# ardaduz/deep-video-mvs

Hardware: AMD Instinct MI355X
Metric: depth frames/sec/GPU @ 320x256x64 planes (fusionnet); rel-L1 vs ref (higher is better)
Workload: dtype f32

## Files before the change

### deep-video-mvs_amd/csrc/direct_conv.hip

```cpp
#include <stdlib.h>

#include "dvmvs_device.h"

namespace dvmvs {

typedef float float4v __attribute__((ext_vector_type(4)));

struct DirectConvArgs {
  const float* x;
  const float* packed;
  const float* bias;
  float* dst;
  float* dst_nhwc;
  long long x_batch_stride, dst_batch_stride;
  int B, C_in, C_out, H, W, OH, OW;
  int act;
  int n_groups;
  int packed_groups;
  int n_chunks;
  int tiles_x;
  int vec4;
};

#ifdef DVMVS_SWEEP_TRACE
// ... 313 lines not shown
#pragma clang fp contract(off)
  if (act == 1) return fmaxf(v, 0.0f);
  if (act == 2 || act == 3) {
    const float s = 1.0f / (1.0f + expf(-v));
    return act == 2 ? s : 1.0f / (p0 * s + p1);
  }
  return v;
}

template <int PX>
__global__ __launch_bounds__(256) void conv_head_kernel(const float* __restrict__ x, const float* __restrict__ w, const float* __restrict__ bias,
                                                        float* __restrict__ dst, long long x_batch_stride, long long dst_batch_stride, int C, int H,
                                                        int W, int act, float p0, float p1) {
  constexpr int SL = 256 / PX;
  __shared__ float s_part[SL][PX];
  const int px = threadIdx.x % PX, slice = threadIdx.x / PX;
  const int HW = H * W;
  const int p = blockIdx.x * PX + px, b = blockIdx.y;
  const int y = p / W, xx = p - y * W;
  const int per = (C + SL - 1) / SL;
  const int c_lo = slice * per, c_hi = min(C, c_lo + per);
  float sum = 0.0f;
  if (p < HW) {
    int off[9];
    bool in[9];
#pragma unroll
    for (int t = 0; t < 9; ++t) {
      const int yy = y + t / 3 - 1, xs = xx + t % 3 - 1;
      in[t] = yy >= 0 && yy < H && xs >= 0 && xs < W;
      off[t] = in[t] ? yy * W + xs : 0;
    }
    const float* xb = x + static_cast<size_t>(b) * x_batch_stride;
#pragma unroll 2
    for (int c = c_lo; c < c_hi; ++c) {
      const float* plane = xb + static_cast<size_t>(c) * HW;
      float v[9];
#pragma unroll
      for (int t = 0; t < 9; ++t) v[t] = in[t] ? plane[off[t]] : 0.0f;
#pragma unroll
      for (int t = 0; t < 9; ++t) sum = fmaf(v[t], w[c * 9 + t], sum);
    }
  }
  s_part[slice][px] = sum;
  __syncthreads();
  if (slice == 0 && p < HW) {
    float total = s_part[0][px];
#pragma unroll
    for (int s = 1; s < SL; ++s) total += s_part[s][px];
    if (bias) total += bias[0];
    dst[static_cast<size_t>(b) * dst_batch_stride + p] = head_activation(total, act, p0, p1);
  }
}

struct DirectConvShape {
  int MW, MT, NT, PW, KS;
};
constexpr DirectConvShape kDcShapes[4] = {{16, 5, 2, 4, 2}, {8, 5, 2, 1, 8}, {16, 5, 1, 1, 8}, {8, 5, 1, 1, 8}};
constexpr int kDcCUs = 256;

inline int direct_conv_choose(int B, int C_in, int C_out, int H, int W, int K, int S) {
  if (B <= 0 || C_in <= 0 || C_out <= 0 || C_out % 16 != 0 || (K != 3 && K != 5) || (S != 1 && S != 2) || H <= 0 || W <= 0) return 0;
  if (S == 2 && (H % 2 != 0 || W % 2 != 0)) return 0;
  const int OH = H / S, OW = W / S;
#if defined(DVMVS_SWEEP_TUNING)
  const char* f = getenv("DVMVS_DC_SHAPE");
  const int forced = f ? atoi(f) : 0;
#else
  const int forced = 0;
#endif
  int best = 0;
  double best_fill = 0.0;
  for (int id = 1; id <= 4; ++id) {
    const DirectConvShape& s = kDcShapes[id - 1];
    const int tile_h = s.PW * (16 / s.MW), tile_w = s.MW * s.MT;
    if (OW % tile_w != 0 || C_out % (16 * s.NT) != 0) continue;
    if (forced == id) return id;
    if (forced) continue;
    const long long groups = static_cast<long long>(OW / tile_w) * ((OH + tile_h - 1) / tile_h) * (C_out / (16 * s.NT)) * B;
    const double fill = static_cast<double>(groups) / static_cast<double>(kDcCUs * ((groups + kDcCUs - 1) / kDcCUs));
    if (fill > best_fill + 1e-9) {
      best_fill = fill;
      best = id;
    }
  }
  return best;
}

template <class Cfg>
int launch_direct_conv(DirectConvArgs a, hipStream_t stream) {
  static bool configured[64] = {};
  constexpr size_t lds = sizeof(float) * Cfg::LDS_FLOATS;
  if (lds > 64 * 1024) {
    int device = 0;
    DVMVS_RETURN_IF_HIP(hipGetDevice(&device));
    const bool tracked = device >= 0 && device < 64;
    if (!tracked || !configured[device]) {
      DVMVS_RETURN_IF_HIP(hipFuncSetAttribute(reinterpret_cast<const void*>(direct_conv_kernel<Cfg>), hipFuncAttributeMaxDynamicSharedMemorySize,
                                              static_cast<int>(lds)));
      if (tracked) configured[device] = true;
    }
  }
  a.n_chunks = (a.n_groups + Cfg::KS * Cfg::G - 1) / (Cfg::KS * Cfg::G);
  a.tiles_x = a.OW / Cfg::TILE_W;
  const int tiles_y = (a.OH + Cfg::TILE_H - 1) / Cfg::TILE_H;
  const dim3 grid(a.tiles_x * tiles_y, a.C_out / (16 * Cfg::NTILE), a.B), block(Cfg::NT);
  hipLaunchKernelGGL((direct_conv_kernel<Cfg>), grid, block, lds, stream, a);
// ... 22 lines not shown

extern "C" size_t dvmvs_direct_conv_packed_bytes(int C_out, int C_in, int kernel_size, int n_tile) {
  if (C_out <= 0 || C_in <= 0 || (n_tile != 1 && n_tile != 2) || C_out % (16 * n_tile) != 0 || (kernel_size != 3 && kernel_size != 5)) return 0;
  const size_t Q = (n_tile * kernel_size + 3) / 4;
  return sizeof(float) * (C_out / (16 * n_tile)) * dvmvs::dc_packed_groups(C_in) * kernel_size * Q * 256;
}

extern "C" int dvmvs_direct_conv_pack(const float* weight, float* packed, int C_out, int C_in, int kernel_size, int n_tile, dvmvs_stream_t stream) {
  if (!weight || !packed) return DVMVS_EINVAL;
  const size_t bytes = dvmvs_direct_conv_packed_bytes(C_out, C_in, kernel_size, n_tile);
  if (bytes == 0) return DVMVS_EUNSUPPORTED;
  const long long total = static_cast<long long>(bytes / sizeof(float));
  hipLaunchKernelGGL(dvmvs::direct_conv_pack_kernel, dim3(static_cast<unsigned int>((total + 255) / 256)), dim3(256), 0, static_cast<hipStream_t>(stream),
                     weight, packed, C_out, C_in, kernel_size, n_tile, dvmvs::dc_packed_groups(C_in), total);
  return dvmvs::launch_status();
}

extern "C" int dvmvs_direct_conv_fwd(const float* x, long long x_batch_stride, const float* packed, int n_tile, const float* bias, float* dst,
                                     long long dst_batch_stride, int B, int C_in, int H, int W, int C_out, int kernel_size, int stride, int activation,
                                     dvmvs_stream_t stream) {
  return dvmvs_direct_conv_dual_fwd(x, x_batch_stride, packed, n_tile, bias, dst, dst_batch_stride, nullptr, B, C_in, H, W, C_out, kernel_size, stride, activation,
                                    stream);
}

extern "C" int dvmvs_direct_conv_dual_fwd(const float* x, long long x_batch_stride, const float* packed, int n_tile, const float* bias, float* dst,
                                          long long dst_batch_stride, float* dst_nhwc, int B, int C_in, int H, int W, int C_out, int kernel_size, int stride,
                                          int activation, dvmvs_stream_t stream) {
  using namespace dvmvs;
  if (!x || !packed || !dst || B <= 0) return DVMVS_EINVAL;
  if (activation != 0 && activation != 1) return DVMVS_EUNSUPPORTED;
  const int id = direct_conv_choose(B, C_in, C_out, H, W, kernel_size, stride);
  if (id == 0) return DVMVS_EUNSUPPORTED;
  if (kDcShapes[id - 1].NT != n_tile) return DVMVS_EINVAL;
  DirectConvArgs a;
  a.x = x; a.packed = packed; a.bias = bias; a.dst = dst; a.dst_nhwc = dst_nhwc;
  a.B = B; a.C_in = C_in; a.C_out = C_out; a.H = H; a.W = W; a.OH = H / stride; a.OW = W / stride;
  a.x_batch_stride = x_batch_stride ? x_batch_stride : static_cast<long long>(C_in) * H * W;
  a.dst_batch_stride = dst_batch_stride ? dst_batch_stride : static_cast<long long>(C_out) * a.OH * a.OW;
  if (a.x_batch_stride < static_cast<long long>(C_in) * H * W || a.dst_batch_stride < static_cast<long long>(C_out) * a.OH * a.OW) return DVMVS_EINVAL;
  if (W % 4 != 0 || a.x_batch_stride % 4 != 0 || (reinterpret_cast<uintptr_t>(x) & 15) != 0) return DVMVS_EUNSUPPORTED;
  if (static_cast<long long>(C_in + 64) * H * W * 4 >= (1LL << 31)) return DVMVS_EUNSUPPORTED;
  a.act = activation;
  a.n_groups = (C_in + 3) / 4;
  a.packed_groups = dc_packed_groups(C_in);
  a.vec4 = (a.OW % 4 == 0 && (a.OH * a.OW) % 4 == 0 && a.dst_batch_stride % 4 == 0 && (reinterpret_cast<uintptr_t>(dst) & 15) == 0) ? 1 : 0;
  a.n_chunks = 0; a.tiles_x = 0;
  hipStream_t s = static_cast<hipStream_t>(stream);
  if (kernel_size == 3) return stride == 1 ? launch_direct_conv_shape<3, 1>(id, a, s) : launch_direct_conv_shape<3, 2>(id, a, s);
  return stride == 1 ? launch_direct_conv_shape<5, 1>(id, a, s) : launch_direct_conv_shape<5, 2>(id, a, s);
}

extern "C" int dvmvs_conv_head_fwd(const float* x, long long x_batch_stride, const float* weight, const float* bias, float* dst,
                                   long long dst_batch_stride, int B, int C_in, int H, int W, int activation, float p0, float p1, dvmvs_stream_t stream) {
  using namespace dvmvs;
  if (!x || !weight || !dst || B <= 0 || C_in <= 0 || H <= 0 || W <= 0) return DVMVS_EINVAL;
  if (activation < 0 || activation > 3) return DVMVS_EINVAL;
  const long long HW = static_cast<long long>(H) * W;
  if (x_batch_stride == 0) x_batch_stride = HW * C_in;
  if (dst_batch_stride == 0) dst_batch_stride = HW;
  hipStream_t s = static_cast<hipStream_t>(stream);
  if (HW >= 16384) {
    hipLaunchKernelGGL((conv_head_kernel<64>), dim3(static_cast<unsigned int>((HW + 63) / 64), B), dim3(256), 0, s, x, weight, bias, dst, x_batch_stride,
                       dst_batch_stride, C_in, H, W, activation, p0, p1);
  } else {
    hipLaunchKernelGGL((conv_head_kernel<16>), dim3(static_cast<unsigned int>((HW + 15) / 16), B), dim3(256), 0, s, x, weight, bias, dst, x_batch_stride,
                       dst_batch_stride, C_in, H, W, activation, p0, p1);
  }
  return launch_status();
}

#ifdef DVMVS_SWEEP_TRACE
extern "C" int dvmvs_debug_direct_conv_trace(unsigned long long* host, int waves) {
  if (waves > dvmvs::kDcTraceWaves) waves = dvmvs::kDcTraceWaves;
  return static_cast<int>(hipMemcpyFromSymbol(host, HIP_SYMBOL(dvmvs::g_dc_trace), sizeof(unsigned long long) * dvmvs::kDcTraceWords * waves));
}
#endif
```

### deep-video-mvs_amd/dvmvs/hip/_capi.py

```python
import ctypes
import os
import threading

import torch

_HERE = os.path.dirname(os.path.abspath(__file__))
LIB_PATH = os.environ.get("DVMVS_HIP_LIB", os.path.normpath(os.path.join(_HERE, "..", "..", "lib", "libdvmvs_hip.so")))

ABI_VERSION = 11
MAX_MEASUREMENTS = 8
MAX_DEPTH_LEVELS = 256
LAYOUT_NCHW, LAYOUT_NHWC = 0, 1

_c_fp = ctypes.c_void_p
_c_fpp = ctypes.POINTER(ctypes.c_void_p)
_c_int = ctypes.c_int
_c_dbl = ctypes.c_double
_c_stream = ctypes.c_void_p
_c_f3 = ctypes.POINTER(ctypes.c_float)

SIGNATURES = {
    "dvmvs_abi_version": (_c_int, []),
    "dvmvs_build_arch": (ctypes.c_char_p, []),
    "dvmvs_error_string": (ctypes.c_char_p, [_c_int]),
    "dvmvs_trace_marker": (_c_int, [_c_stream]),
    "dvmvs_host_pointer_device_visible": (_c_int, [ctypes.c_void_p]),
    "dvmvs_cost_volume_workspace_bytes": (ctypes.c_size_t, [_c_int, _c_int, _c_int, _c_int, _c_int]),
    "dvmvs_sweep_matrices": (_c_int, [_c_fp, _c_fpp, _c_fp, _c_fp, _c_fp, _c_int, _c_int, _c_stream]),
    "dvmvs_cost_volume_fwd": (_c_int, [_c_fp, _c_fpp, _c_fp, _c_fp, _c_fp,
                                       _c_int, _c_int, _c_int, _c_int, _c_int, _c_int,
                                       _c_dbl, _c_dbl, _c_int, _c_int, _c_int, _c_fp, ctypes.c_size_t, _c_stream]),
    "dvmvs_sweep_plan_stats": (_c_int, [_c_fp, _c_fp, _c_int, _c_int, _c_int, _c_int, _c_int, _c_dbl, _c_dbl, _c_int,
                                        ctypes.POINTER(ctypes.c_longlong)]),
    "dvmvs_sweep_select_variant": (_c_int, [_c_fp, _c_fp, _c_int, _c_int, _c_int, _c_int, _c_int, _c_dbl, _c_dbl]),
    "dvmvs_sweep_work_list_bytes": (ctypes.c_size_t, [_c_int, _c_int, _c_int, _c_int]),
    "dvmvs_sweep_work_list": (_c_int, [_c_fp, _c_fp, _c_int, _c_int, _c_int, _c_int, _c_int, _c_dbl, _c_dbl, _c_int, _c_fp, ctypes.c_size_t]),
    "dvmvs_sweep_plan": (_c_int, [_c_fp, _c_fp, _c_int, _c_int, _c_int, _c_int, _c_int, _c_dbl, _c_dbl, _c_int, _c_fp, ctypes.c_size_t]),
    "dvmvs_sweep_plan6": (_c_int, [_c_fp, _c_fp, _c_int, _c_int, _c_int, _c_int, _c_int, _c_dbl, _c_dbl, _c_fp, ctypes.c_size_t]),
    "dvmvs_nchw_to_nhwc": (_c_int, [_c_fp, _c_fp, _c_int, _c_int, _c_int, _c_int, _c_stream]),
    "dvmvs_copy_batch": (_c_int, [_c_fpp, _c_fpp, ctypes.POINTER(ctypes.c_longlong), _c_int, _c_stream]),
    "dvmvs_sweep_mfma_estimate": (_c_int, [_c_fp, _c_fp, _c_int, _c_int, _c_int, _c_int, _c_int, _c_dbl, _c_dbl, ctypes.POINTER(ctypes.c_double)]),
    "dvmvs_cost_volume_planned_fwd": (_c_int, [_c_fp, _c_fpp, _c_fp, _c_fp, _c_fp,
                                               _c_int, _c_int, _c_int, _c_int, _c_int, _c_int,
                                               _c_dbl, _c_dbl, _c_int, _c_int, _c_int, _c_fp, ctypes.c_size_t, _c_fp, _c_stream]),
    "dvmvs_cost_volume_bwd": (_c_int, [_c_fp, _c_fp, _c_fpp, _c_fp, _c_fp, _c_fp, _c_fpp,
                                       _c_int, _c_int, _c_int, _c_int, _c_int, _c_int,
                                       _c_dbl, _c_dbl, _c_stream]),
    "dvmvs_hidden_warp_fwd": (_c_int, [_c_fp, _c_fp, _c_fp, _c_fp, _c_fp, _c_int, _c_int, _c_int, _c_int, _c_int, _c_stream]),
    "dvmvs_hidden_warp_bwd": (_c_int, [_c_fp, _c_fp, _c_fp, _c_fp, _c_fp, _c_int, _c_int, _c_int, _c_int, _c_stream]),
    "dvmvs_relative_pose": (_c_int, [_c_fp, _c_fp, _c_fp, _c_int, _c_stream]),
    "dvmvs_lstm_gates_fwd": (_c_int, [_c_fp, _c_fp, _c_fp, _c_fp, _c_int, _c_int, _c_int, _c_int, _c_stream]),
    "dvmvs_lstm_gates_bwd": (_c_int, [_c_fp, _c_fp, _c_fp, _c_fp, _c_fp, _c_fp, _c_int, _c_int, _c_int, _c_int, _c_stream]),
    "dvmvs_lstm_gates_partials_fwd": (_c_int, [_c_fp, _c_int, _c_fp, _c_fp, _c_fp, _c_int, _c_int, _c_int, _c_int, _c_stream]),
    "dvmvs_bottleneck_conv_packed_bytes": (ctypes.c_size_t, [_c_int, _c_int]),
    "dvmvs_bottleneck_conv_pack": (_c_int, [_c_fp, _c_fp, _c_int, _c_int, _c_stream]),
    "dvmvs_bottleneck_conv_splits": (_c_int, [_c_int] * 6),
    "dvmvs_bottleneck_conv_fwd": (_c_int, [_c_fp, _c_fp, _c_fp] + [_c_int] * 6 + [_c_stream]),
    "dvmvs_bottleneck_conv_up2x_fwd": (_c_int, [_c_fp, _c_fp, _c_fp] + [_c_int] * 5 + [_c_stream]),
    "dvmvs_direct_conv_tile": (_c_int, [_c_int] * 7),
    "dvmvs_direct_conv_packed_bytes": (ctypes.c_size_t, [_c_int] * 4),
    "dvmvs_direct_conv_pack": (_c_int, [_c_fp, _c_fp, _c_int, _c_int, _c_int, _c_int, _c_stream]),
    "dvmvs_direct_conv_fwd": (_c_int, [_c_fp, ctypes.c_longlong, _c_fp, _c_int, _c_fp, _c_fp, ctypes.c_longlong] + [_c_int] * 8 + [_c_stream]),
    "dvmvs_direct_conv_dual_fwd": (_c_int, [_c_fp, ctypes.c_longlong, _c_fp, _c_int, _c_fp, _c_fp, ctypes.c_longlong, _c_fp] + [_c_int] * 8 + [_c_stream]),
    "dvmvs_pointwise_conv_supported": (_c_int, [_c_int] * 7),
    "dvmvs_pointwise_conv_packed_bytes": (ctypes.c_size_t, [_c_int] * 2),
    "dvmvs_pointwise_conv_pack": (_c_int, [_c_fp, _c_fp, _c_int, _c_int, _c_stream]),
    "dvmvs_pointwise_conv_fwd": (_c_int, [_c_fp, ctypes.c_longlong, _c_fp, _c_fp, _c_fp, ctypes.c_longlong, _c_int, _c_fp, ctypes.c_longlong] + [_c_int] * 7 + [_c_stream]),
    "dvmvs_conv_head_fwd": (_c_int, [_c_fp, ctypes.c_longlong, _c_fp, _c_fp, _c_fp, ctypes.c_longlong] + [_c_int] * 5 + [ctypes.c_float, ctypes.c_float, _c_stream]),
    "dvmvs_partial_sums_bias_act_fwd": (_c_int, [_c_fp, _c_int, _c_fp, ctypes.c_longlong, _c_fp, _c_int, _c_int, _c_int, _c_int, _c_stream]),
    "dvmvs_depth_reproject_fwd": (_c_int, [_c_fp, _c_fp, _c_fp, _c_fp, _c_fp, _c_fp, _c_int,
                                           _c_int, _c_int, _c_int, _c_stream]),
    "dvmvs_bias_act_fwd": (_c_int, [_c_fp, _c_fp, ctypes.c_longlong, _c_fp, _c_fp, _c_int, _c_int, _c_int, _c_int, _c_int, _c_int,
                                    ctypes.c_float, ctypes.c_float, _c_stream]),
    "dvmvs_bias_act_inplace": (_c_int, [_c_fp, _c_fp, _c_fp, _c_int, _c_int, _c_int, _c_int, _c_int, _c_int, _c_stream]),
    "dvmvs_conv_bias_act_fwd": (_c_int, [_c_fp, _c_fp, _c_fp, _c_fp, ctypes.c_longlong] + [_c_int] * 9 + [_c_stream]),
    "dvmvs_upsample2x_fwd": (_c_int, [_c_fp, _c_fp, ctypes.c_longlong, _c_fp, _c_int, _c_int, _c_int, _c_int, _c_int, _c_stream]),
    "dvmvs_upsample2x_pair_fwd": (_c_int, [_c_fp, _c_fp, ctypes.c_longlong, _c_int, _c_fp, _c_fp, ctypes.c_longlong, _c_fp, _c_int, _c_int, _c_int, _c_int, _c_int, _c_stream]),
    "dvmvs_upsample2x_bwd": (_c_int, [_c_fp, _c_fp, _c_int, _c_int, _c_int, _c_int, _c_stream]),
    "dvmvs_depthwise_conv_bwd_workspace_bytes": (ctypes.c_size_t, [_c_int] * 6),
    "dvmvs_depthwise_conv_bwd": (_c_int, [_c_fp, _c_fp, _c_fp, _c_fp, _c_fp, _c_fp, _c_int, _c_int, _c_int, _c_int, _c_int, _c_int, _c_stream]),
    "dvmvs_depth_reproject_lowres_fwd": (_c_int, [_c_fp, _c_fp, _c_fp, _c_fp, _c_fp, _c_fp, _c_int, _c_int, _c_int, _c_int, _c_stream]),
    "dvmvs_depth_reproject_estimate_fwd": (_c_int, [_c_fp, _c_fp, _c_fp, _c_fp, _c_fp, _c_fp, _c_int, _c_int, _c_int, _c_int, _c_stream]),
    "dvmvs_tsdf_integrate": (_c_int, [_c_fp, _c_fp, _c_fp, _c_int, _c_int, _c_int, ctypes.c_float, ctypes.c_float, ctypes.c_float,
                                      ctypes.c_float, _c_fp, _c_fp, _c_fp, _c_fp, _c_int, _c_int, ctypes.c_float, ctypes.c_float, _c_stream]),
    "dvmvs_marching_cubes_workspace_bytes": (ctypes.c_size_t, [_c_int, _c_int, _c_int]),
    "dvmvs_marching_cubes_count": (_c_int, [_c_fp, _c_int, _c_int, _c_int, ctypes.c_float, _c_fp, ctypes.c_size_t, _c_fp, _c_stream]),
    "dvmvs_marching_cubes_emit": (_c_int, [_c_fp, _c_fp, _c_int, _c_int, _c_int, ctypes.c_float, ctypes.c_float, ctypes.c_float,
                                           ctypes.c_float, ctypes.c_float, _c_fp, _c_fp, _c_fp, _c_fp, _c_fp, ctypes.c_longlong,
                                           ctypes.c_longlong, _c_stream]),
    "dvmvs_depthwise_conv_fwd": (_c_int, [_c_fp, _c_fp, _c_fp, _c_fp, _c_int, _c_fp, _c_int, _c_int, _c_int, _c_int, _c_int, _c_int, _c_int,
                                          _c_stream]),
    "dvmvs_rgb_sweep_fwd": (_c_int, [_c_fp, _c_fpp, _c_fp, _c_fp, _c_fp, _c_int, _c_int, _c_int, _c_int, _c_int, _c_int,
                                     _c_dbl, _c_dbl, _c_int, _c_int, _c_int, _c_stream]),
    "dvmvs_gp_filter_step": (_c_int, [_c_fp, _c_fp, _c_fp, _c_int, _c_dbl, _c_dbl, _c_dbl, _c_dbl, _c_dbl, _c_dbl, _c_int, _c_stream]),
    "dvmvs_dps_volume_fwd": (_c_int, [_c_fp, _c_fp, _c_fp, _c_fp, _c_fp, _c_fp, _c_int, _c_int, _c_int, _c_int, _c_int, _c_dbl, _c_stream]),
    "dvmvs_dps_regress_fwd": (_c_int, [_c_fp, _c_fp, _c_fp, _c_int, _c_int, _c_int, _c_int, _c_int, _c_int, _c_dbl, _c_stream]),
    "dvmvs_preprocess_rgb_fwd": (_c_int, [_c_fp, _c_fp, _c_int, _c_int, _c_int, ctypes.c_longlong, _c_int, _c_int, _c_int, _c_int,
                                          ctypes.c_longlong, _c_dbl, _c_f3, _c_f3, _c_int, _c_stream]),
    "dvmvs_preprocess_depth_fwd": (_c_int, [_c_fp, _c_fp, _c_int, _c_int, _c_int, _c_int, _c_int, _c_int, _c_int, _c_dbl, _c_stream]),
}

ADDED_WITHIN_ABI = ("dvmvs_preprocess_rgb_fwd", "dvmvs_preprocess_depth_fwd")

_lib = None
_lock = threading.Lock()


def lib():
    global _lib
    if _lib is not None:
        return _lib
    with _lock:
        if _lib is not None:
            return _lib
        if not os.path.exists(LIB_PATH):
            raise RuntimeError(
                f"dvmvs HIP library not found at {LIB_PATH}. Build it with `make -C deep-video-mvs_amd/csrc` "
                f"(or __graft_entry__.build()). The plane-sweep ops have no CPU / eager fallback.")
        handle = ctypes.CDLL(LIB_PATH)
        missing = [name for name in ADDED_WITHIN_ABI if not hasattr(handle, name)]
        if missing:
# ... 29 lines not shown
```

### deep-video-mvs_amd/dvmvs/hip/ops.py

```python
import ctypes
import os
from typing import Optional, Sequence, Tuple

import torch
from torch import Tensor

from dvmvs.hip import _capi

__all__ = ["cost_volume", "sweep_matrices", "hidden_warp", "relative_pose", "lstm_gates", "depth_reproject", "depth_reproject_lowres",
           "bias_act_", "upsample2x", "depthwise_conv", "rgb_sweep", "gp_filter_step", "dps_volume", "dps_regress", "preprocess_rgb",
           "preprocess_depth"]


COST_VOLUME_TWO_PASS = os.environ.get("DVMVS_COST_VOLUME_TWO_PASS", "1") == "1"


_workspaces = {}


def sweep_workspace(device, B, M, H, W, D):
    device = torch.device(device)
    index = device.index if device.index is not None else torch.cuda.current_device()
    key = (index, B, M, H, W, D)
    entry = _workspaces.get(key)
# ... 497 lines not shown
def _depthwise_train_setup(ctx, inputs, output):
    x, weight, stride = inputs
    ctx.stride = stride
    ctx.save_for_backward(x, weight)


def _depthwise_train_backward(ctx, grad):
    x, weight = ctx.saved_tensors
    need_input, need_weight = ctx.needs_input_grad[0], ctx.needs_input_grad[1]
    gx, gw = depthwise_conv_bwd(grad, x, weight, ctx.stride, need_input, need_weight)
    return (gx if need_input else None), (gw if need_weight else None), None


torch.library.register_autograd("dvmvs::depthwise_conv_train", _depthwise_train_backward, setup_context=_depthwise_train_setup)


@torch.library.custom_op("dvmvs::depthwise_conv", mutates_args=(), device_types="cuda")
def depthwise_conv(x: Tensor, weight: Tensor, bias: Tensor, stride: int, activation: int, pre_bias: Tensor, pre_relu: bool) -> Tensor:
    _dev_f32("depthwise_conv", x, weight)
    x, weight = x.contiguous(), weight.contiguous()
    B, C, H, W = x.shape
    k = weight.shape[-1]
    if tuple(weight.shape) != (C, 1, k, k):
        raise ValueError(f"dvmvs::depthwise_conv: weight {tuple(weight.shape)} is not depthwise for {C} channels")
    pad = k // 2
    OH, OW = (H + 2 * pad - k) // stride + 1, (W + 2 * pad - k) // stride + 1
    out = torch.empty((B, C, OH, OW), dtype=torch.float32, device=x.device)
    with torch.cuda.device(x.device):
        if pre_bias.numel() not in (0, C):
            raise ValueError(f"dvmvs::depthwise_conv: pre_bias has {pre_bias.numel()} entries for {C} channels")
        rc = _capi.lib().dvmvs_depthwise_conv_fwd(_ptr(x), _ptr(weight), _ptr(bias.contiguous()) if bias.numel() else None,
                                                  _ptr(pre_bias.contiguous()) if pre_bias.numel() else None, int(bool(pre_relu)), _ptr(out),
                                                  B, C, H, W, k, int(stride), int(activation), _stream(x))
    _capi.check(rc, "dvmvs_depthwise_conv_fwd")
    return out


@depthwise_conv.register_fake
def _(x, weight, bias, stride, activation, pre_bias, pre_relu):
    B, C, H, W = x.shape
    k = weight.shape[-1]
    pad = k // 2
    return x.new_empty((B, C, (H + 2 * pad - k) // stride + 1, (W + 2 * pad - k) // stride + 1))


@depthwise_conv.register_kernel("cpu")
def _(x, weight, bias, stride, activation, pre_bias, pre_relu):
    _no_cpu("depthwise_conv")


ACTIVATION_SIGMOID_TO_DEPTH = 3


def _slice_batch_stride(name, dst, B, C, H, W):
    if dst.device.type != "cuda" or dst.dtype != torch.float32:
        raise TypeError(f"dvmvs::{name}: destination must be a float32 HIP tensor")
    if tuple(dst.shape) != (B, C, H, W) or dst.stride(3) != 1 or dst.stride(2) != W or dst.stride(1) != H * W:
        raise ValueError(f"dvmvs::{name}: destination {tuple(dst.shape)} / strides {dst.stride()} is not a channel slice of a "
                         f"contiguous NCHW buffer for [{B},{C},{H},{W}]")
    return dst.stride(0) if B > 1 else C * H * W


def bias_act_into(x: Tensor, dst: Tensor, bias, activation: int, residual=None, residual_mode: int = RESIDUAL_NONE, p0: float = 0.0,
                  p1: float = 0.0) -> Tensor:
    _dev_f32("bias_act_into", x)
    if not x.is_contiguous() or x.dim() != 4:
        raise ValueError("dvmvs::bias_act_into: expected a contiguous NCHW source")
    B, C, H, W = x.shape
    stride = _slice_batch_stride("bias_act_into", dst, B, C, H, W)
    if bias is not None and bias.numel() not in (0, C):
        raise ValueError(f"dvmvs::bias_act_into: bias has {bias.numel()} entries for {C} channels")
    res_ptr = None
    if residual_mode != RESIDUAL_NONE:
        want = (B, C, H, W) if residual_mode == RESIDUAL_SAME else (B, C, H // 2, W // 2)
        if tuple(residual.shape) != want or not residual.is_contiguous():
            raise ValueError(f"dvmvs::bias_act_into: residual {tuple(residual.shape)} does not match {want} (contiguous)")
        res_ptr = _ptr(residual)
    with torch.cuda.device(x.device):
        rc = _capi.lib().dvmvs_bias_act_fwd(_ptr(x), _ptr(dst), stride, _ptr(bias) if bias is not None and bias.numel() else None, res_ptr,
                                            int(residual_mode), B, C, H, W, int(activation), float(p0), float(p1), _stream(x))
    _capi.check(rc, "dvmvs_bias_act_fwd")
    return dst


EUNSUPPORTED = -2


def conv_bias_act_into(x: Tensor, weight: Tensor, bias: Tensor, dst, stride: int, padding: int, activation: int):
    _dev_f32("conv_bias_act_into", x, weight, bias)
    if activation not in (ACTIVATIONS["none"], ACTIVATIONS["relu"]):
        raise ValueError("dvmvs::conv_bias_act_into: activation must be none or relu")
    x, weight = x.contiguous(), weight.contiguous()
    B, Cin, H, W = x.shape
    Cout, Cin_w, K, K2 = weight.shape
    if Cin_w != Cin or K != K2 or bias.numel() != Cout:
        raise ValueError(f"dvmvs::conv_bias_act_into: weight {tuple(weight.shape)} / bias {bias.numel()} do not fit input {tuple(x.shape)}")
    Ho, Wo = (H + 2 * padding - K) // stride + 1, (W + 2 * padding - K) // stride + 1
    if dst is None:
        dst = torch.empty(B, Cout, Ho, Wo, device=x.device, dtype=torch.float32)
    batch_stride = _slice_batch_stride("conv_bias_act_into", dst, B, Cout, Ho, Wo)
    with torch.cuda.device(x.device):
        rc = _capi.lib().dvmvs_conv_bias_act_fwd(_ptr(x), _ptr(weight), _ptr(bias), _ptr(dst), batch_stride, B, Cin, H, W, Cout, K,
                                                 int(stride), int(padding), int(activation), _stream(x))
    if rc == EUNSUPPORTED:
        return None
    _capi.check(rc, "dvmvs_conv_bias_act_fwd")
# ... 126 lines not shown
            raise ValueError("dvmvs::direct_conv_into: dst_nhwc must be a dense channels-last tensor of the output's shape")
    with torch.cuda.device(x.device):
        rc = _capi.lib().dvmvs_direct_conv_dual_fwd(_ptr(x), 0, _ptr(packed), int(n_tile), _ptr(bias) if bias is not None and bias.numel() else None,
                                                    _ptr(dst), batch_stride, _ptr(dst_nhwc) if dst_nhwc is not None else None, B, C_in, H, W, int(C_out),
                                                    int(kernel_size), int(stride), int(activation), _stream(x))
    _capi.check(rc, "dvmvs_direct_conv_dual_fwd")
    return dst


def pointwise_conv_supported(B: int, C_in: int, H: int, W: int, C_out: int, activation: int, residual_mode: int) -> bool:
    return bool(_capi.lib().dvmvs_pointwise_conv_supported(int(B), int(C_in), int(H), int(W), int(C_out), int(activation), int(residual_mode)))


def pointwise_conv_pack(weight: Tensor) -> Tensor:
    _dev_f32("pointwise_conv_pack", weight)
    if weight.dim() not in (2, 4) or (weight.dim() == 4 and tuple(weight.shape[2:]) != (1, 1)):
        raise ValueError(f"dvmvs::pointwise_conv_pack: need a [C_out,C_in,1,1] weight, got {tuple(weight.shape)}")
    C_out, C_in = int(weight.shape[0]), int(weight.shape[1])
    nbytes = _capi.lib().dvmvs_pointwise_conv_packed_bytes(C_out, C_in)
    packed = torch.empty(nbytes // 4, device=weight.device, dtype=torch.float32)
    with torch.cuda.device(weight.device):
        rc = _capi.lib().dvmvs_pointwise_conv_pack(_ptr(weight.contiguous()), _ptr(packed), C_out, C_in, _stream(weight))
    _capi.check(rc, "dvmvs_pointwise_conv_pack")
    return packed


def pointwise_conv_into(x: Tensor, packed: Tensor, bias, dst: Tensor, C_out: int, activation: int, residual=None, residual_mode: int = 0,
                        splits: int = 0) -> Tensor:
    _dev_f32("pointwise_conv_into", x, packed, dst)
    if x.dim() != 4 or not x.is_contiguous():
        raise ValueError("dvmvs::pointwise_conv_into: expected a contiguous NCHW input")
    B, C_in, H, W = x.shape
    C_out = int(C_out)
    if packed.numel() * 4 != _capi.lib().dvmvs_pointwise_conv_packed_bytes(C_out, C_in):
        raise ValueError(f"dvmvs::pointwise_conv_into: the packed weights are not those of a {C_in} -> {C_out} layer")
    batch_stride = _slice_batch_stride("pointwise_conv_into", dst, B, C_out, H, W)
    if bias is not None and bias.numel() not in (0, C_out):
        raise ValueError(f"dvmvs::pointwise_conv_into: bias has {bias.numel()} entries for {C_out} channels")
    residual_stride = 0
    if residual_mode:
        _dev_f32("pointwise_conv_into", residual)
        shape = (B, C_out, H, W) if residual_mode == 1 else (B, C_out, H // 2, W // 2)
        if tuple(residual.shape) != shape:
            raise ValueError(f"dvmvs::pointwise_conv_into: residual of shape {tuple(residual.shape)}, mode {residual_mode} expects {shape}")
        residual_stride = _slice_batch_stride("pointwise_conv_into", residual, *shape)
    with torch.cuda.device(x.device):
        rc = _capi.lib().dvmvs_pointwise_conv_fwd(_ptr(x), 0, _ptr(packed), _ptr(bias) if bias is not None and bias.numel() else None,
                                                  _ptr(residual) if residual_mode else None, residual_stride, int(residual_mode), _ptr(dst), batch_stride,
                                                  B, C_in, H, W, C_out, int(activation), int(splits), _stream(x))
    _capi.check(rc, "dvmvs_pointwise_conv_fwd")
    return dst


def conv_head_into(x: Tensor, weight: Tensor, bias, dst: Tensor, activation: int = 0, p0: float = 0.0, p1: float = 0.0) -> Tensor:
    _dev_f32("conv_head_into", x, weight, dst)
    if x.dim() != 4 or not x.is_contiguous() or tuple(weight.shape) != (1, x.shape[1], 3, 3) or not weight.is_contiguous():
        raise ValueError(f"dvmvs::conv_head_into: expected a contiguous NCHW input and a [1,{x.shape[1]},3,3] weight, got {tuple(x.shape)}, {tuple(weight.shape)}")
    B, C_in, H, W = x.shape
    batch_stride = _slice_batch_stride("conv_head_into", dst, B, 1, H, W)
    with torch.cuda.device(x.device):
        rc = _capi.lib().dvmvs_conv_head_fwd(_ptr(x), 0, _ptr(weight), _ptr(bias) if bias is not None and bias.numel() else None, _ptr(dst),
                                             batch_stride, B, C_in, H, W, int(activation), float(p0), float(p1), _stream(x))
    _capi.check(rc, "dvmvs_conv_head_fwd")
    return dst


def lstm_gates_partials_into(conv_partials: Tensor, n_partials: int, c_state: Tensor, h_state: Tensor) -> None:
    _dev_f32("lstm_gates_partials_into", conv_partials, c_state, h_state)
    B, hidden, H, W = c_state.shape
    if conv_partials.numel() < n_partials * B * 4 * hidden * H * W or tuple(h_state.shape) != tuple(c_state.shape):
        raise ValueError("dvmvs::lstm_gates_partials_into: shapes do not match")
    if not (conv_partials.is_contiguous() and c_state.is_contiguous() and h_state.is_contiguous()):
        raise ValueError("dvmvs::lstm_gates_partials_into: expected contiguous tensors")
    with torch.cuda.device(c_state.device):
        rc = _capi.lib().dvmvs_lstm_gates_partials_fwd(_ptr(conv_partials), int(n_partials), _ptr(c_state), _ptr(h_state), _ptr(c_state), B, hidden, H, W,
                                                       _stream(c_state))
    _capi.check(rc, "dvmvs_lstm_gates_partials_fwd")


def hidden_warp_into(image_src: Tensor, depth_dst: Tensor, src_trans_dst: Tensor, camera_matrix: Tensor, zero_invalid: bool, dst: Tensor) -> Tensor:
    _dev_f32("hidden_warp_into", image_src, depth_dst, src_trans_dst, camera_matrix, dst)
    B, C, H, W = image_src.shape
    if not (image_src.is_contiguous() and dst.is_contiguous() and tuple(dst.shape) == (B, C, H, W)):
        raise ValueError("dvmvs::hidden_warp_into: source and destination must be contiguous [B,C,H,W]")
    with torch.cuda.device(image_src.device):
        rc = _capi.lib().dvmvs_hidden_warp_fwd(_ptr(image_src), _ptr(depth_dst.contiguous()), _ptr(src_trans_dst.contiguous()),
                                               _ptr(camera_matrix.contiguous()), _ptr(dst), B, C, H, W, int(bool(zero_invalid)), _stream(image_src))
    _capi.check(rc, "dvmvs_hidden_warp_fwd")
    return dst


def depth_reproject_lowres_into(transformation: Tensor, previous_depth: Tensor, full_K: Tensor, half_K: Tensor, zbuffer: Tensor, out_lowres: Tensor,
                                factor: int) -> Tensor:
    _dev_f32("depth_reproject_lowres_into", transformation, previous_depth, full_K, half_K, zbuffer, out_lowres)
    B, one, Hf, Wf = previous_depth.shape
    if one != 1 or zbuffer.numel() != B * (Hf // 2) * (Wf // 2) or not zbuffer.is_contiguous() or not out_lowres.is_contiguous() or \
            out_lowres.numel() != B * ((Hf // 2) // factor) * ((Wf // 2) // factor):
        raise ValueError("dvmvs::depth_reproject_lowres_into: buffer shapes do not match the previous depth")
    with torch.cuda.device(previous_depth.device):
        rc = _capi.lib().dvmvs_depth_reproject_lowres_fwd(_ptr(transformation.contiguous()), _ptr(previous_depth.contiguous()), _ptr(full_K.contiguous()),
                                                          _ptr(half_K.contiguous()), _ptr(zbuffer), _ptr(out_lowres), int(factor), B, Hf, Wf,
                                                          _stream(previous_depth))
    _capi.check(rc, "dvmvs_depth_reproject_lowres_fwd")
    return out_lowres


def depth_reproject_estimate_into(transformation: Tensor, previous_depth: Tensor, full_K: Tensor, half_K: Tensor, estimate: Tensor,
                                  estimate_to_clear: Optional[Tensor], factor: int) -> Tensor:
    _dev_f32("depth_reproject_estimate_into", transformation, previous_depth, full_K, half_K, estimate)
    B, one, Hf, Wf = previous_depth.shape
    shape = (B, 1, Hf // 2 // factor, Wf // 2 // factor)
    if one != 1 or tuple(estimate.shape) != shape or not estimate.is_contiguous() or not previous_depth.is_contiguous() or \
            (estimate_to_clear is not None and (tuple(estimate_to_clear.shape) != shape or not estimate_to_clear.is_contiguous() or
                                                estimate_to_clear.data_ptr() == estimate.data_ptr())):
        raise ValueError("dvmvs::depth_reproject_estimate_into: expected contiguous [B,1,H,W] depth and distinct [B,1,H/2/f,W/2/f] estimate buffers")
    with torch.cuda.device(previous_depth.device):
        rc = _capi.lib().dvmvs_depth_reproject_estimate_fwd(_ptr(transformation.contiguous()), _ptr(previous_depth), _ptr(full_K.contiguous()),
# ... 252 lines not shown
```

### include/dvmvs_hip.h

```cpp
#ifndef DVMVS_HIP_H
#define DVMVS_HIP_H

#include <stddef.h>
#include <stdint.h>

#ifdef __cplusplus
extern "C" {
#endif

#define DVMVS_ABI_VERSION 11
#define DVMVS_MAX_MEASUREMENTS 8
#define DVMVS_MAX_DEPTH_LEVELS 256

#define DVMVS_LAYOUT_NCHW 0
#define DVMVS_LAYOUT_NHWC 1

#define DVMVS_EINVAL (-1)
#define DVMVS_EUNSUPPORTED (-2)
#define DVMVS_ELIBRARY (-3)

typedef void* dvmvs_stream_t;

int dvmvs_abi_version(void);
const char* dvmvs_build_arch(void);
// ... 32 lines not shown
                                  double min_depth, double max_depth, int dot_product, int variant, int image2_layout,
                                  float* workspace, size_t workspace_bytes, const unsigned int* work_list, dvmvs_stream_t stream);

int dvmvs_cost_volume_bwd(const float* grad_cost, const float* image1, const float* const* image2s,
                          const float* Hm, const float* kt, float* grad_image1, float* const* grad_image2s,
                          int B, int M, int C, int H, int W, int D,
                          double min_depth, double max_depth, dvmvs_stream_t stream);

int dvmvs_hidden_warp_fwd(const float* image_src, const float* depth_dst, const float* src_trans_dst,
                          const float* camera_matrix, float* out, int B, int C, int H, int W,
                          int zero_invalid, dvmvs_stream_t stream);

int dvmvs_hidden_warp_bwd(const float* grad_out, const float* depth_dst, const float* src_trans_dst,
                          const float* camera_matrix, float* grad_src, int B, int C, int H, int W,
                          dvmvs_stream_t stream);

int dvmvs_relative_pose(const float* a, const float* c, float* out, int B, dvmvs_stream_t stream);

int dvmvs_lstm_gates_fwd(const float* combined_conv, const float* c_cur, float* h_next, float* c_next,
                         int B, int hidden, int H, int W, dvmvs_stream_t stream);

int dvmvs_lstm_gates_bwd(const float* grad_h, const float* grad_c, const float* combined_conv,
                         const float* c_cur, float* grad_cc, float* grad_c_cur,
                         int B, int hidden, int H, int W, dvmvs_stream_t stream);

int dvmvs_upsample2x_bwd(const float* grad_out, float* grad_in, int B, int C, int H, int W, dvmvs_stream_t stream);
size_t dvmvs_depthwise_conv_bwd_workspace_bytes(int B, int C, int H, int W, int kernel_size, int stride);
int dvmvs_depthwise_conv_bwd(const float* grad_out, const float* in, const float* weight, float* grad_in, float* grad_weight,
                             float* workspace, int B, int C, int H, int W, int kernel_size, int stride, dvmvs_stream_t stream);

size_t dvmvs_bottleneck_conv_packed_bytes(int C_out, int C_in);
int dvmvs_bottleneck_conv_pack(const float* weight, float* packed, int C_out, int C_in, dvmvs_stream_t stream);
int dvmvs_bottleneck_conv_splits(int B, int C_out, int C_in, int H_in, int W_in, int stride);
int dvmvs_bottleneck_conv_fwd(const float* x, const float* packed, float* partials, int B, int C_in, int H_in, int W_in, int C_out,
                              int stride, dvmvs_stream_t stream);
int dvmvs_bottleneck_conv_up2x_fwd(const float* x, const float* packed, float* partials, int B, int C_in, int H_in, int W_in, int C_out,
                                   dvmvs_stream_t stream);
int dvmvs_partial_sums_bias_act_fwd(const float* partials, int n_partials, float* dst, long long dst_batch_stride, const float* bias,
                                    int B, int C, int HW, int activation, dvmvs_stream_t stream);
int dvmvs_lstm_gates_partials_fwd(const float* conv_partials, int n_partials, const float* c_cur, float* h_next, float* c_next,
                                  int B, int hidden, int H, int W, dvmvs_stream_t stream);

int dvmvs_direct_conv_tile(int B, int C_in, int H, int W, int C_out, int kernel_size, int stride);
size_t dvmvs_direct_conv_packed_bytes(int C_out, int C_in, int kernel_size, int n_tile);
int dvmvs_direct_conv_pack(const float* weight, float* packed, int C_out, int C_in, int kernel_size, int n_tile, dvmvs_stream_t stream);
int dvmvs_direct_conv_fwd(const float* x, long long x_batch_stride, const float* packed, int n_tile, const float* bias, float* dst,
                          long long dst_batch_stride, int B, int C_in, int H, int W, int C_out, int kernel_size, int stride, int activation,
                          dvmvs_stream_t stream);
int dvmvs_direct_conv_dual_fwd(const float* x, long long x_batch_stride, const float* packed, int n_tile, const float* bias, float* dst,
                               long long dst_batch_stride, float* dst_nhwc, int B, int C_in, int H, int W, int C_out, int kernel_size, int stride,
                               int activation, dvmvs_stream_t stream);
int dvmvs_conv_head_fwd(const float* x, long long x_batch_stride, const float* weight, const float* bias, float* dst,
                        long long dst_batch_stride, int B, int C_in, int H, int W, int activation, float p0, float p1, dvmvs_stream_t stream);

int dvmvs_pointwise_conv_supported(int B, int C_in, int H, int W, int C_out, int activation, int residual_mode);
size_t dvmvs_pointwise_conv_packed_bytes(int C_out, int C_in);
int dvmvs_pointwise_conv_pack(const float* weight, float* packed, int C_out, int C_in, dvmvs_stream_t stream);
int dvmvs_pointwise_conv_fwd(const float* x, long long x_batch_stride, const float* packed, const float* bias, const float* residual,
                             long long residual_batch_stride, int residual_mode, float* dst, long long dst_batch_stride, int B, int C_in,
                             int H, int W, int C_out, int activation, int splits, dvmvs_stream_t stream);

int dvmvs_depth_reproject_fwd(const float* transformation, const float* previous_depth, const float* full_K,
                              const float* half_K, float* out, float* out_lowres, int lowres_factor,
                              int B, int full_height, int full_width, dvmvs_stream_t stream);
int dvmvs_depth_reproject_lowres_fwd(const float* transformation, const float* previous_depth, const float* full_K,
                                     const float* half_K, float* zbuffer, float* out_lowres, int lowres_factor,
                                     int B, int full_height, int full_width, dvmvs_stream_t stream);

int dvmvs_depth_reproject_estimate_fwd(const float* transformation, const float* previous_depth, const float* full_K,
                                       const float* half_K, float* estimate, float* estimate_to_clear, int lowres_factor,
                                       int B, int full_height, int full_width, dvmvs_stream_t stream);

int dvmvs_bias_act_fwd(const float* x, float* dst, long long dst_batch_stride, const float* bias, const float* residual,
                       int residual_mode, int B, int C, int H, int W, int activation, float p0, float p1, dvmvs_stream_t stream);
int dvmvs_bias_act_inplace(float* x, const float* bias, const float* residual, int residual_mode, int B, int C, int H, int W,
                           int activation, dvmvs_stream_t stream);
int dvmvs_upsample2x_fwd(const float* in, float* out, long long out_batch_stride, const float* pre_bias, int pre_activation,
                         int B, int C, int H, int W, dvmvs_stream_t stream);
int dvmvs_upsample2x_pair_fwd(const float* in1, float* out1, long long out1_batch_stride, int C1, const float* in2, float* out2,
                              long long out2_batch_stride, const float* pre_bias2, int pre_activation2, int C2, int B, int H, int W,
                              dvmvs_stream_t stream);
int dvmvs_conv_bias_act_fwd(const float* x, const float* weight, const float* bias, float* out, long long out_batch_stride,
                            int B, int Cin, int H, int W, int Cout, int K, int stride, int padding, int activation, dvmvs_stream_t stream);
int dvmvs_depthwise_conv_fwd(const float* in, const float* weight, const float* bias, const float* pre_bias, int pre_relu, float* out,
                             int B, int C, int H, int W, int kernel_size, int stride, int activation, dvmvs_stream_t stream);

int dvmvs_tsdf_integrate(float* tsdf_vol, float* weight_vol, float* color_vol, int dim_x, int dim_y, int dim_z,
                         float origin_x, float origin_y, float origin_z, float voxel_size, const float* cam_intr,
                         const float* cam_pose, const float* color_im, const float* depth_im, int im_h, int im_w,
                         float trunc_margin, float obs_weight, dvmvs_stream_t stream);

size_t dvmvs_marching_cubes_workspace_bytes(int X, int Y, int Z);
int dvmvs_marching_cubes_count(const float* vol, int X, int Y, int Z, float level, void* workspace, size_t workspace_bytes,
                               long long* counts_dev, dvmvs_stream_t stream);
int dvmvs_marching_cubes_emit(const float* vol, const float* color_vol, int X, int Y, int Z, float level, float ox, float oy, float oz,
                              float voxel_size, void* workspace, float* verts, float* normals, unsigned char* colors, int* faces,
                              long long V, long long F, dvmvs_stream_t stream);

int dvmvs_rgb_sweep_fwd(const float* image1, const float* const* image2s, const float* Hm, const float* kt, float* out,
                        int B, int M, int C, int H, int W, int D, double min_depth, double max_depth, int Cout,
                        int channel_offset, int copy_image, dvmvs_stream_t stream);
int dvmvs_gp_filter_step(double* state, const float* y, float* z, int N, double a00, double a01, double a10, double a11,
                         double k0, double k1, int reset, dvmvs_stream_t stream);

int dvmvs_dps_volume_fwd(const float* ref, const float* meas, const float* pose, const float* K, const float* Kinv, float* out,
                         int B, int C, int h, int w, int nlabel, double mindepth, dvmvs_stream_t stream);
// ... 14 lines not shown
```

Measured before the change: 1414.

## Add quad-pixel row kernel for 3x3 single-output conv head

Adds a conv head kernel in which each thread computes four horizontally adjacent outputs. It loads a 128-bit center vector plus two edge scalars per row, using buffer loads whose out-of-range offsets return zero, so the per-tap bounds checks go away. Weights are staged in LDS, and channel loads are double-buffered across a split-channel reduction. The old one-pixel kernel stays as a fallback and can be forced through a path argument. The cost is more registers per thread and a dependence on alignment and width conditions.

```diff
diff --git a/deep-video-mvs_amd/csrc/direct_conv.hip b/deep-video-mvs_amd/csrc/direct_conv.hip
--- a/deep-video-mvs_amd/csrc/direct_conv.hip
+++ b/deep-video-mvs_amd/csrc/direct_conv.hip
@@ -389,6 +389,127 @@
   }
 }
 
+constexpr unsigned int kHeadOutOfRange = 0x80000000u;
+constexpr unsigned int kHeadDeadChannel = 0x40000000u;
+constexpr int kHeadMaxChannels = 1024;
+
+struct HeadChannel {
+  float4v m[3];
+  float l[3], r[3];
+};
+
+template <int SL>
+__global__ __launch_bounds__(64) void conv_head_rows_kernel(const float* __restrict__ x, const float* __restrict__ w, const float* __restrict__ bias,
+                                                            float* __restrict__ dst, long long x_batch_stride, long long dst_batch_stride, int C, int H,
+                                                            int W, int act, float p0, float p1) {
+#pragma clang fp contract(off)
+  constexpr int QB = 64 / SL, U = 4;
+  extern __shared__ __attribute__((aligned(16))) float s_head[];
+  float4v* s_part = reinterpret_cast<float4v*>(s_head);
+  float* s_w = s_head + 256;
+  const int tid = threadIdx.x, ql = tid % QB, slice = tid / QB;
+  const int QW = W >> 2, n_quads = H * QW, HW = H * W;
+  const int q = blockIdx.x * QB + ql, b = blockIdx.y;
+  const bool live = q < n_quads;
+  const int y = q / QW, x0 = 4 * (q - y * QW);
+  const int per = (C + SL - 1) / SL;
+  const int c_lo = slice * per, c_hi = min(C, c_lo + per);
+
+  unsigned int off[3][3];
+#pragma unroll
+  for (int r = 0; r < 3; ++r) {
+    const int yy = y + r - 1;
+    const bool row_in = live && yy >= 0 && yy < H;
+    const unsigned int base = 4u * static_cast<unsigned int>(yy * W + x0);
+    off[r][0] = (row_in && x0 > 0) ? base - 4u : kHeadOutOfRange;
+    off[r][1] = row_in ? base : kHeadOutOfRange;
+    off[r][2] = (row_in && x0 + 4 < W) ? base + 16u : kHeadOutOfRange;
+  }
+  const __amdgpu_buffer_rsrc_t x_resource = __builtin_amdgcn_make_buffer_rsrc(
+      (void*)(as_global(x) + static_cast<size_t>(b) * x_batch_stride), 0, static_cast<int>(sizeof(float) * static_cast<unsigned int>(C) * HW), 0x00020000);
+
+  auto load = [&](HeadChannel(&buf)[U], int j0) __attribute__((always_inline)) {
+#pragma unroll
+    for (int u = 0; u < U; ++u) {
+      const int c = c_lo + j0 + u;
+      const unsigned int cb = c < c_hi ? 4u * static_cast<unsigned int>(c) * static_cast<unsigned int>(HW) : kHeadDeadChannel;
+#pragma unroll
+      for (int r = 0; r < 3; ++r) {
+        buf[u].l[r] = __builtin_bit_cast(float, __builtin_amdgcn_raw_buffer_load_b32(x_resource, static_cast<int>(off[r][0] + cb), 0, 0));
+        buf[u].m[r] = __builtin_bit_cast(float4v, __builtin_amdgcn_raw_buffer_load_b128(x_resource, static_cast<int>(off[r][1] + cb), 0, 0));
+        buf[u].r[r] = __builtin_bit_cast(float, __builtin_amdgcn_raw_buffer_load_b32(x_resource, static_cast<int>(off[r][2] + cb), 0, 0));
+      }
+    }
+  };
+  float acc[4] = {0.0f, 0.0f, 0.0f, 0.0f};
+  auto multiply = [&](const HeadChannel(&buf)[U], int j0) __attribute__((always_inline)) {
+#pragma unroll
+    for (int u = 0; u < U; ++u) {
+      const int c = c_lo + j0 + u;
+      if (c < c_hi) {
+        float wt[9];
+#pragma unroll
+        for (int t = 0; t < 9; ++t) wt[t] = s_w[c * 9 + t];
+#pragma unroll
+        for (int t = 0; t < 9; ++t) {
+          const int r = t / 3, k = t % 3;
+#pragma unroll
+          for (int e = 0; e < 4; ++e) {
+            const int col = e + k - 1;
+            const float v = col < 0 ? buf[u].l[r] : (col > 3 ? buf[u].r[r] : buf[u].m[r][col]);
+            acc[e] = fmaf(v, wt[t], acc[e]);
+          }
+        }
+      }
+    }
+  };
+
+  HeadChannel first[U], second[U];
+  load(first, 0);
+  {
+    const int n = C * 9;
+    const int n4 = (reinterpret_cast<uintptr_t>(w) & 15) == 0 ? n >> 2 : 0;
+    for (int i = tid; i < n4; i += 64) reinterpret_cast<float4v*>(s_w)[i] = reinterpret_cast<const float4v*>(w)[i];
+    for (int i = 4 * n4 + tid; i < n; i += 64) s_w[i] = w[i];
+  }
+  __syncthreads();
+  for (int j0 = 0; j0 < per; j0 += 2 * U) {
+    if (j0 + U < per) load(second, j0 + U);
+    multiply(first, j0);
+    if (j0 + 2 * U < per) load(first, j0 + 2 * U);
+    if (j0 + U < per) multiply(second, j0 + U);
+  }
+
+  float4v sum;
+#pragma unroll
+  for (int e = 0; e < 4; ++e) sum[e] = acc[e];
+  s_part[slice * QB + ql] = sum;
+  __syncthreads();
+  if (slice == 0 && live) {
+    float4v total = s_part[ql];
+#pragma unroll
+    for (int s = 1; s < SL; ++s) {
+      const float4v part = s_part[s * QB + ql];
+#pragma unroll
+      for (int e = 0; e < 4; ++e) total[e] += part[e];
+    }
+    if (bias) {
+      const float bv = bias[0];
+#pragma unroll
+      for (int e = 0; e < 4; ++e) total[e] += bv;
+    }
+#pragma unroll
+    for (int e = 0; e < 4; ++e) total[e] = head_activation(total[e], act, p0, p1);
+    *reinterpret_cast<float4v*>(dst + static_cast<size_t>(b) * dst_batch_stride + static_cast<size_t>(y) * W + x0) = total;
+  }
+}
+
+inline bool conv_head_rows_taken(const float* x, long long x_batch_stride, const float* dst, long long dst_batch_stride, int B, int C, int H, int W) {
+  const long long HW = static_cast<long long>(H) * W;
+  return W % 4 == 0 && (reinterpret_cast<uintptr_t>(x) & 15) == 0 && (reinterpret_cast<uintptr_t>(dst) & 15) == 0 && x_batch_stride % 4 == 0 &&
+         dst_batch_stride % 4 == 0 && C <= kHeadMaxChannels && HW * C * 4 < (1LL << 30) && B <= 65535;
+}
+
 struct DirectConvShape {
   int MW, MT, NT, PW, KS;
 };
@@ -517,13 +638,38 @@
 
 extern "C" int dvmvs_conv_head_fwd(const float* x, long long x_batch_stride, const float* weight, const float* bias, float* dst,
                                    long long dst_batch_stride, int B, int C_in, int H, int W, int activation, float p0, float p1, dvmvs_stream_t stream) {
+  return dvmvs_conv_head_path_fwd(x, x_batch_stride, weight, bias, dst, dst_batch_stride, B, C_in, H, W, activation, p0, p1, 0, stream);
+}
+
+extern "C" int dvmvs_conv_head_rows_path(const float* x, long long x_batch_stride, const float* dst, long long dst_batch_stride, int B, int C_in,
+                                         int H, int W) {
+  if (!x || !dst || B <= 0 || C_in <= 0 || H <= 0 || W <= 0) return 0;
+  const long long HW = static_cast<long long>(H) * W;
+  return dvmvs::conv_head_rows_taken(x, x_batch_stride ? x_batch_stride : HW * C_in, dst, dst_batch_stride ? dst_batch_stride : HW, B, C_in, H, W) ? 1 : 0;
+}
+
+extern "C" int dvmvs_conv_head_path_fwd(const float* x, long long x_batch_stride, const float* weight, const float* bias, float* dst,
+                                        long long dst_batch_stride, int B, int C_in, int H, int W, int activation, float p0, float p1, int path,
+                                        dvmvs_stream_t stream) {
   using namespace dvmvs;
   if (!x || !weight || !dst || B <= 0 || C_in <= 0 || H <= 0 || W <= 0) return DVMVS_EINVAL;
-  if (activation < 0 || activation > 3) return DVMVS_EINVAL;
+  if (activation < 0 || activation > 3 || path < 0 || path > 1) return DVMVS_EINVAL;
   const long long HW = static_cast<long long>(H) * W;
   if (x_batch_stride == 0) x_batch_stride = HW * C_in;
   if (dst_batch_stride == 0) dst_batch_stride = HW;
   hipStream_t s = static_cast<hipStream_t>(stream);
+  if (path == 0 && conv_head_rows_taken(x, x_batch_stride, dst, dst_batch_stride, B, C_in, H, W)) {
+    const unsigned int quads = static_cast<unsigned int>(HW / 4);
+    const size_t lds = sizeof(float) * (256 + static_cast<size_t>(C_in) * 9);
+    if (HW >= 16384) {
+      hipLaunchKernelGGL((conv_head_rows_kernel<4>), dim3((quads + 15) / 16, B), dim3(64), lds, s, x, weight, bias, dst, x_batch_stride, dst_batch_stride, C_in,
+                         H, W, activation, p0, p1);
+    } else {
+      hipLaunchKernelGGL((conv_head_rows_kernel<16>), dim3((quads + 3) / 4, B), dim3(64), lds, s, x, weight, bias, dst, x_batch_stride, dst_batch_stride, C_in,
+                         H, W, activation, p0, p1);
+    }
+    return launch_status();
+  }
   if (HW >= 16384) {
     hipLaunchKernelGGL((conv_head_kernel<64>), dim3(static_cast<unsigned int>((HW + 63) / 64), B), dim3(256), 0, s, x, weight, bias, dst, x_batch_stride,
                        dst_batch_stride, C_in, H, W, activation, p0, p1);
diff --git a/deep-video-mvs_amd/dvmvs/hip/_capi.py b/deep-video-mvs_amd/dvmvs/hip/_capi.py
--- a/deep-video-mvs_amd/dvmvs/hip/_capi.py
+++ b/deep-video-mvs_amd/dvmvs/hip/_capi.py
@@ -67,6 +67,8 @@
     "dvmvs_pointwise_conv_pack": (_c_int, [_c_fp, _c_fp, _c_int, _c_int, _c_stream]),
     "dvmvs_pointwise_conv_fwd": (_c_int, [_c_fp, ctypes.c_longlong, _c_fp, _c_fp, _c_fp, ctypes.c_longlong, _c_int, _c_fp, ctypes.c_longlong] + [_c_int] * 7 + [_c_stream]),
     "dvmvs_conv_head_fwd": (_c_int, [_c_fp, ctypes.c_longlong, _c_fp, _c_fp, _c_fp, ctypes.c_longlong] + [_c_int] * 5 + [ctypes.c_float, ctypes.c_float, _c_stream]),
+    "dvmvs_conv_head_path_fwd": (_c_int, [_c_fp, ctypes.c_longlong, _c_fp, _c_fp, _c_fp, ctypes.c_longlong] + [_c_int] * 5 + [ctypes.c_float, ctypes.c_float, _c_int, _c_stream]),
+    "dvmvs_conv_head_rows_path": (_c_int, [_c_fp, ctypes.c_longlong, _c_fp, ctypes.c_longlong] + [_c_int] * 4),
     "dvmvs_partial_sums_bias_act_fwd": (_c_int, [_c_fp, _c_int, _c_fp, ctypes.c_longlong, _c_fp, _c_int, _c_int, _c_int, _c_int, _c_stream]),
     "dvmvs_depth_reproject_fwd": (_c_int, [_c_fp, _c_fp, _c_fp, _c_fp, _c_fp, _c_fp, _c_int,
                                            _c_int, _c_int, _c_int, _c_stream]),
diff --git a/deep-video-mvs_amd/dvmvs/hip/ops.py b/deep-video-mvs_amd/dvmvs/hip/ops.py
--- a/deep-video-mvs_amd/dvmvs/hip/ops.py
+++ b/deep-video-mvs_amd/dvmvs/hip/ops.py
@@ -573,6 +573,9 @@
 ACTIVATION_SIGMOID_TO_DEPTH = 3
 
 
+CONV_HEAD_PATHS = {"auto": 0, "one_pixel": 1}
+
+
 def _slice_batch_stride(name, dst, B, C, H, W):
     if dst.device.type != "cuda" or dst.dtype != torch.float32:
         raise TypeError(f"dvmvs::{name}: destination must be a float32 HIP tensor")
@@ -805,17 +808,24 @@
     return dst
 
 
-def conv_head_into(x: Tensor, weight: Tensor, bias, dst: Tensor, activation: int = 0, p0: float = 0.0, p1: float = 0.0) -> Tensor:
+def conv_head_into(x: Tensor, weight: Tensor, bias, dst: Tensor, activation: int = 0, p0: float = 0.0, p1: float = 0.0, path: str = "auto") -> Tensor:
     _dev_f32("conv_head_into", x, weight, dst)
     if x.dim() != 4 or not x.is_contiguous() or tuple(weight.shape) != (1, x.shape[1], 3, 3) or not weight.is_contiguous():
         raise ValueError(f"dvmvs::conv_head_into: expected a contiguous NCHW input and a [1,{x.shape[1]},3,3] weight, got {tuple(x.shape)}, {tuple(weight.shape)}")
+    if path not in CONV_HEAD_PATHS:
+        raise ValueError(f"dvmvs::conv_head_into: path must be one of {sorted(CONV_HEAD_PATHS)}, got {path!r}")
     B, C_in, H, W = x.shape
     batch_stride = _slice_batch_stride("conv_head_into", dst, B, 1, H, W)
     with torch.cuda.device(x.device):
-        rc = _capi.lib().dvmvs_conv_head_fwd(_ptr(x), 0, _ptr(weight), _ptr(bias) if bias is not None and bias.numel() else None, _ptr(dst),
-                                             batch_stride, B, C_in, H, W, int(activation), float(p0), float(p1), _stream(x))
-    _capi.check(rc, "dvmvs_conv_head_fwd")
+        rc = _capi.lib().dvmvs_conv_head_path_fwd(_ptr(x), 0, _ptr(weight), _ptr(bias) if bias is not None and bias.numel() else None, _ptr(dst),
+                                                  batch_stride, B, C_in, H, W, int(activation), float(p0), float(p1), CONV_HEAD_PATHS[path], _stream(x))
+    _capi.check(rc, "dvmvs_conv_head_path_fwd")
     return dst
+
+
+def conv_head_rows_path(x: Tensor, dst: Tensor) -> bool:
+    B, C_in, H, W = x.shape
+    return bool(_capi.lib().dvmvs_conv_head_rows_path(_ptr(x), 0, _ptr(dst), _slice_batch_stride("conv_head_rows_path", dst, B, 1, H, W), B, C_in, H, W))
 
 
 def lstm_gates_partials_into(conv_partials: Tensor, n_partials: int, c_state: Tensor, h_state: Tensor) -> None:
diff --git a/include/dvmvs_hip.h b/include/dvmvs_hip.h
--- a/include/dvmvs_hip.h
+++ b/include/dvmvs_hip.h
@@ -108,6 +108,10 @@
                                int activation, dvmvs_stream_t stream);
 int dvmvs_conv_head_fwd(const float* x, long long x_batch_stride, const float* weight, const float* bias, float* dst,
                         long long dst_batch_stride, int B, int C_in, int H, int W, int activation, float p0, float p1, dvmvs_stream_t stream);
+int dvmvs_conv_head_path_fwd(const float* x, long long x_batch_stride, const float* weight, const float* bias, float* dst,
+                             long long dst_batch_stride, int B, int C_in, int H, int W, int activation, float p0, float p1, int path,
+                             dvmvs_stream_t stream);
+int dvmvs_conv_head_rows_path(const float* x, long long x_batch_stride, const float* dst, long long dst_batch_stride, int B, int C_in, int H, int W);
 
 int dvmvs_pointwise_conv_supported(int B, int C_in, int H, int W, int C_out, int activation, int residual_mode);
 size_t dvmvs_pointwise_conv_packed_bytes(int C_out, int C_in);
```

Result: no change. 1404 (-0.7%).
